# POSTECH-CVLab/PyTorch-StudioGAN

Hardware: AMD Instinct MI355X
Metric: images/sec (G+D step) BigGAN ImageNet-128 bs256 (higher is better)
Workload: dtype bf16

## Files before the change

include/sgamd.h:

```cpp
#ifndef SGAMD_H
#define SGAMD_H
#include <stdint.h>
#ifdef __cplusplus
extern "C" {
#endif

typedef void* sg_stream_t;

#define SG_DTYPE_F32 0
#define SG_DTYPE_BF16 1
#define SG_DTYPE_F64 2

#define SG_PIX_RELU 1
#define SG_PIX_UPSAMPLE 2
#define SG_PIX_QUAD 4
#define SG_PIX_TRANSPOSED 8
#define SG_EPI_OUT_F32 1
#define SG_EPI_ATOMIC 2
#define SG_EPI_POOL 4
#define SG_EPI_RELU 8
#define SG_EPI_RES_F32 16

const char* sg_last_error(void);
int sg_version(void);
// ... 167 lines not shown
  float* sigma;
  float* u_snap; float* v_snap;
  void* w_fwd;
  void* w_dgrad;
  float* w_f32;
  int rows, cols;
  int Cin, RS;
  int do_power_iter;
  int apply_sn;
  int rows_pad;
  long long work_off;
  int trans;
  int dgrad_noflip;
  int Cin_pad;
} sg_sn_layer;
int sg_sn_forward(int dtype, const sg_sn_layer* layers_dev, const sg_sn_layer* layers_host, int n, float eps, float* work, long long work_floats, sg_stream_t s);

typedef struct {
  const float* dwt;
  const float* w;
  const float* u; const float* v; const float* sigma;
  float* dw;
  int rows, cols, Cin, RS, natural, apply_sn, trans;
  int Cin_pad;
} sg_sn_bwd_layer;
int sg_sn_backward(const sg_sn_bwd_layer* layers_dev, const sg_sn_bwd_layer* layers_host, int n, float* work, long long work_floats, sg_stream_t s);

int sg_embedding_fwd(const float* table, const int64_t* idx, float* out, int B, int dim, int num, sg_stream_t s);
int sg_embedding_bwd(const float* dout, const int64_t* idx, float* dtable, int B, int dim, int num, sg_stream_t s);
int sg_relu_sum_hw_fwd(int dtype, const void* x, float* h, int B, int HW, int C, sg_stream_t s);
int sg_relu_sum_hw_bwd(int dtype, const void* x, const float* dh, void* dx, int B, int HW, int C, sg_stream_t s);
int sg_pd_head_fwd(const float* h, const float* w1, const float* b1, const float* emb, float* adv, int B, int C, sg_stream_t s);
int sg_pd_head_bwd(const float* h, const float* w1, const float* emb, const float* dadv, float* dh, float* dw1, float* db1,
                   float* demb, int B, int C, sg_stream_t s);
int sg_loss_d(int kind, const float* real, const float* fake, int B, float* loss, float* d_real, float* d_fake, sg_stream_t s);
int sg_loss_g(int kind, const float* fake, int B, float* loss, float* d_fake, sg_stream_t s);

int sg_interp_rows(const float* real, const float* fake, const float* alpha, float* out, int B, long long n, sg_stream_t s);
int sg_gp_fwd(int kind, const float* grads, int B, long long n, float* norms, float* loss, sg_stream_t s);
int sg_gp_bwd(int kind, const float* grads, const float* norms, const float* gout, float* dgrads, int B, long long n, sg_stream_t s);
int sg_masked_sum_hw(int dtype, const void* t, const void* x, float* out, int B, int HW, int C, sg_stream_t s);

int sg_attn_fwd_flash_ok(int B, int HW, int HW4, int Dp, int Cg);
int sg_attn_fwd_fused(const void* theta, const void* phi, const void* g, float* lse, void* O, float* O32, int B, int HW, int HW4, int Dp, int Cg, sg_stream_t s);
int sg_attn_bwd_fused_ok(int B, int HW, int HW4, int Dp, int Cg);
int sg_attn_bwd_fused(const void* theta, const void* phi, const void* g, const void* dO, const float* O32, const float* lse, float* delta, void* dtheta, void* dphi,
                      void* dg, int B, int HW, int HW4, int Dp, int Cg, sg_stream_t s);

int sg_attn_proj_ok(int B, int H, int W, int C, int ldx, int Dp, int Cg);
int sg_attn_proj_fwd(const void* x, int ldx, const void* w_theta, const void* w_phi, const void* w_g, void* theta, void* phi, void* g,
                     uint8_t* idx_phi, uint8_t* idx_g, int B, int H, int W, int C, int Dp, int Cg, int relu, sg_stream_t s);
int sg_attn_proj_bwd_data(const void* dtheta, const void* dphi, const void* dg, const uint8_t* idx_phi, const uint8_t* idx_g, const void* wd_theta,
                          const void* wd_phi, const void* wd_g, const void* res, void* dx, int B, int H, int W, int C, int Dp, int Cg, sg_stream_t s);

int sg_slice_up_fwd(int dtype, const void* x, void* y, int N, int Hs, int Ws, int ldx, int C, int up, sg_stream_t s);
int sg_slice_up_bwd(int dtype, const void* dy, void* dx, int N, int Hs, int Ws, int ldx, int C, int up, sg_stream_t s);
int sg_copy_channels(int dtype, const void* src, int ld_src, void* dst, int ld_dst, long long rows, int C, sg_stream_t s);

int sg_adam_ema(float* p, const float* g, float* m, float* v, float* ema, long long n, float lr, float beta1, float beta2,
                float eps, float wd, int step, float ema_decay, float grad_scale, sg_stream_t s);
int sg_ema_lerp(const float* src, float* ema, long long n, float decay, sg_stream_t s);

int sg_lecam(const float* real, const float* fake, int B, float ema_real, float ema_fake, float* loss, float* d_real, float* d_fake, sg_stream_t s);
int sg_u8_to_nhwc(int dtype, const uint8_t* x, const uint8_t* flip, void* y, int N, int H, int W, int cpad, sg_stream_t s);

int sg_quantize_resize_normalize(int dtype, const float* x, void* out, uint8_t* quant_out, int N, int C, int H, int W,
                                 int OH, int OW, int quantize, sg_stream_t s);
int sg_quantize_resize_normalize_ms(int dtype, const float* x, void* out, uint8_t* quant_out, int N, int C, int H, int W,
                                    int OH, int OW, int quantize, const float* mean, const float* std, sg_stream_t s);
int sg_pool2d(int dtype, const void* x, void* y, int N, int H, int W, int C, int k, int stride, int pad, int mode, int ldy, int c_off, sg_stream_t s);
int sg_pil_resize_normalize(int dtype, const float* x, void* out, float* tmp, int N, int C, int H, int W, int OH, int OW,
                            const int* bounds_h, const double* kk_h, int ksize_h, const int* bounds_v, const double* kk_v, int ksize_v,
                            int quantize, sg_stream_t s);
int sg_pil_resize_normalize_ms(int dtype, const float* x, void* out, float* tmp, int N, int C, int H, int W, int OH, int OW,
                               const int* bounds_h, const double* kk_h, int ksize_h, const int* bounds_v, const double* kk_v, int ksize_v,
                               int quantize, const float* mean, const float* std, sg_stream_t s);
int sg_global_avgpool(int dtype, const void* x, float* y, int N, int HW, int C, sg_stream_t s);
int sg_topk_hits(const float* scores, int ld, int ncls, const int64_t* labels, int k, int N, uint8_t* hits, sg_stream_t s);
int sg_topk_select(const float* x, int n, int k, float* vals, int* idx, sg_stream_t s);
int sg_topk_scatter(const float* g, const int* idx, int k, float* dx, int n, sg_stream_t s);
int sg_feat_moments_accumulate(const float* f, int n, int C, double* sum_f, double* sum_ff, sg_stream_t s);
int sg_gather_images_u8(const uint8_t* src, const int64_t* idx, const uint8_t* flip, uint8_t* dst, int B, int H, int W,
                        const int64_t* lab_src, int64_t* lab_dst, sg_stream_t s);
int sg_row_normalize_fwd(const float* x, float* y, float* inv, int rows, int cols, float eps, sg_stream_t s);
int sg_row_normalize_bwd(const float* y, const float* inv, const float* dy, float* dx, int rows, int cols, sg_stream_t s);
int sg_row_dot(const float* a, const float* b, float* p, int rows, int cols, sg_stream_t s);
int sg_row_scale(const float* g, const float* x, float* out, int rows, int cols, int accumulate, sg_stream_t s);
int sg_class_loss(int kind, const float* z, const int64_t* label, int rows, int cols, float* row_loss, float* loss, float* dz, sg_stream_t s);
int sg_contrastive_loss(int kind, const float* S, const float* p, const int64_t* label, int B, float temperature, float m_p,
                        float* row_loss, float* loss, float* dS, float* dp, sg_stream_t s);
int sg_gather_cols(const float* z, const int64_t* label, int rows, int cols, float* out, sg_stream_t s);
int sg_scatter_cols(const float* g, const int64_t* label, int rows, int cols, float* dz, sg_stream_t s);
int sg_layernorm_rows(int out_dtype, const float* x, long long pitch, const float* gamma, const float* beta, void* y, long long ldo, int rows, int C,
                      float eps, sg_stream_t s);
int sg_vit_tokens(const float* patch, const float* cls, const float* pos, float* x, int B, int N, int C, sg_stream_t s);
int sg_gelu_f32(const float* x, float* y, long long n, sg_stream_t s);
int sg_tok_gemm(int epi, const void* a, int lda, const void* w, const float* bias, void* out, int ldo, int M, int N, int K, sg_stream_t s);
int sg_mha_fwd_ok(int B, int N, int H, int D);
int sg_mha_fwd(const void* qkv, void* out, int B, int N, int H, int D, float scale, sg_stream_t s);
long long sg_tok_gemm_launches(void);
long long sg_mha_launches(void);

int sg_row_sqnorm(const float* f, int n, int C, float* sq, sg_stream_t s);
int sg_kth_smallest_rows(const float* D, long long ld, int rows, int cols, int k, const float* row_add, float* out, sg_stream_t s);
int sg_prdc_rows(const float* D, long long ld, int rows, int cols, const float* row_add, const float* r2_row, const float* r2_col,
                 int* col_cnt, uint8_t* row_any, float* row_min, sg_stream_t s);
// ... 62 lines not shown
```

pytorch-studiogan_amd/_lib.py:

```python
import ctypes as C
import os
import subprocess
import sys

import torch

_HERE = os.path.dirname(os.path.abspath(__file__))
LIB_PATH = os.path.join(_HERE, "libsgamd.so")
if os.environ.get("SG_LIBSGAMD"):
    LIB_PATH = os.path.abspath(os.environ["SG_LIBSGAMD"])
CSRC = os.path.join(_HERE, "csrc")

F32, BF16, F64 = 0, 1, 2
PIX_RELU, PIX_UPSAMPLE, PIX_QUAD, PIX_TRANSPOSED = 1, 2, 4, 8
Q_POOL, Q_UP = 0, 1
EPI_OUT_F32, EPI_ATOMIC, EPI_POOL, EPI_RELU, EPI_RES_F32 = 1, 2, 4, 8, 16

_vp, _i, _f, _ll = C.c_void_p, C.c_int, C.c_float, C.c_longlong


class ConvFwdDesc(C.Structure):
    _fields_ = [("dtype", _i), ("N", _i), ("Hs", _i), ("Ws", _i), ("C", _i), ("ldx", _i), ("Ho", _i), ("Wo", _i), ("Cout", _i),
                ("R", _i), ("S", _i), ("stride", _i), ("pad_h", _i), ("pad_w", _i), ("pix_flags", _i), ("epi_flags", _i),
                ("alpha", _f), ("beta", _f), ("x", _vp), ("w", _vp), ("bias", _vp), ("res", _vp), ("mask", _vp), ("out", _vp),
# ... 96 lines not shown
    "sg_gemm": [C.POINTER(GemmDesc), _vp],
    "sg_nchw_to_nhwc": [_i, _vp, _vp, _i, _i, _i, _i, _i, _vp],
    "sg_nhwc_to_nchw": [_i, _vp, _vp, _i, _i, _i, _i, _i, _i, _vp],
    "sg_nchw_grad_to_nhwc": [_i, _vp, _vp, _vp, _i, _i, _i, _i, _i, _i, _vp],
    "sg_avgpool2_fwd": [_i, _vp, _vp, _i, _i, _i, _i, _vp],
    "sg_avgpool2_bwd": [_i, _vp, _vp, _i, _i, _i, _i, _vp],
    "sg_maxpool2_fwd": [_i, _vp, _i, _vp, _i, _vp, _i, _i, _i, _i, _vp],
    "sg_maxpool2_bwd": [_i, _vp, _i, _vp, _vp, _i, _i, _i, _i, _i, _vp],
    "sg_softmax_rows": [_i, _vp, _vp, _ll, _i, _vp],
    "sg_softmax_rows_bwd": [_i, _vp, _vp, _vp, _ll, _i, _vp],
    "sg_axpby": [_i, _vp, _vp, _ll, _f, _f, _vp],
    "sg_convert": [_i, _i, _vp, _vp, _ll, _vp],
    "sg_add_relu": [_i, _vp, _vp, _vp, _ll, _vp],
    "sg_relu_mask": [_i, _vp, _vp, _vp, _ll, _vp],
    "sg_dot": [_i, _vp, _vp, _ll, _vp, _f, _vp, _vp],
    "sg_colsum": [_i, _vp, _i, _vp, _i, _ll, _i, _vp, _f, _vp],
    "sg_bn_partial_stats": [_i, _vp, _i, _ll, _i, _vp, _vp],
    "sg_bn_finalize": [_vp, C.c_double, _i, _f, _f, _vp, _vp, _vp, _vp, _vp],
    "sg_comm_unique_id": [_vp],
    "sg_comm_init_rank": [_vp, _i, _i, C.POINTER(_vp)],
    "sg_comm_size": [_vp, C.POINTER(_i)],
    "sg_comm_destroy": [_vp],
    "sg_allreduce_flat": [_vp, _vp, _ll, _i, _vp],
    "sg_bn_stats_sync": [_i, _vp, _i, _ll, _i, _vp, _vp, _f, _f, _vp, _vp, _vp, _vp, _vp],
    "sg_set_f32_mode": [_i],
    "sg_get_f32_mode": [],
    "sg_f32_split_launches": [_i],
    "sg_reduce_scatter_flat": [_vp, _vp, _ll, _vp],
    "sg_allgather_flat": [_vp, _vp, _ll, _vp],
    "sg_p2p_create": [_i, _i, _ll, C.POINTER(_vp), _vp],
    "sg_p2p_connect": [_vp, _vp],
    "sg_p2p_destroy": [_vp],
    "sg_p2p_timeouts": [_vp, C.POINTER(_i)],
    "sg_p2p_allreduce_f64": [_vp, _vp, _i, _vp],
    "sg_bn_finalize_p2p": [_vp, _vp, C.c_double, _i, _f, _f, _vp, _vp, _vp, _vp, _vp],
    "sg_bn_stats_sync_p2p": [_i, _vp, _i, _ll, _i, _vp, _vp, _f, _f, _vp, _vp, _vp, _vp, _vp],
    "sg_bn_from_running": [_vp, _vp, _i, _f, _vp, _vp, _vp],
    "sg_bn_apply": [_i, _vp, _vp, _i, _ll, _i, _vp, _vp, _vp, _vp, _i, _i, _vp],
    "sg_bn_bwd_reduce": [_i, _vp, _vp, _i, _ll, _i, _vp, _vp, _vp, _vp, _i, _i, _vp, _vp],
    "sg_bn_bwd_finalize": [_vp, _i, _i, _vp, _i, _vp, _vp, _vp, _vp],
    "sg_bn_bwd_apply": [_i, _vp, _vp, _vp, _i, _ll, _i, _vp, _vp, _vp, _vp, _i, _i, _vp, C.c_double, _i, _vp],
    "sg_bn_bwd_apply_res": [_i, _vp, _vp, _vp, _i, _ll, _i, _vp, _vp, _vp, _vp, _i, _i, _vp, C.c_double, _i, _vp, _vp],
    "sg_bn_bwd2_reduce": [_i, _vp, _vp, _vp, _i, _ll, _i, _vp, _vp, _vp, _vp, _i, _vp, _vp],
    "sg_bn_bwd2_finalize": [_vp, _i, _i, _vp, _vp],
    "sg_bn_bwd2_dgain": [_vp, _vp, C.c_double, _vp, _i, _i, _vp, _vp],
    "sg_bn_bwd2_apply": [_i, _vp, _vp, _vp, _vp, _vp, _i, _ll, _i, _vp, _vp, _vp, _vp, _i, _vp, C.c_double, _i, _vp],
    "sg_attn_fwd_flash_ok": [_i, _i, _i, _i, _i],
    "sg_attn_fwd_fused": [_vp, _vp, _vp, _vp, _vp, _vp, _i, _i, _i, _i, _i, _vp],
    "sg_attn_bwd_fused_ok": [_i, _i, _i, _i, _i],
    "sg_attn_bwd_fused": [_vp, _vp, _vp, _vp, _vp, _vp, _vp, _vp, _vp, _vp, _i, _i, _i, _i, _i, _vp],
    "sg_attn_proj_ok": [_i, _i, _i, _i, _i, _i, _i],
    "sg_attn_proj_fwd": [_vp, _i, _vp, _vp, _vp, _vp, _vp, _vp, _vp, _vp, _i, _i, _i, _i, _i, _i, _i, _vp],
    "sg_attn_proj_bwd_data": [_vp, _vp, _vp, _vp, _vp, _vp, _vp, _vp, _vp, _vp, _i, _i, _i, _i, _i, _i, _vp],
    "sg_slice_up_fwd": [_i, _vp, _vp, _i, _i, _i, _i, _i, _i, _vp],
    "sg_slice_up_bwd": [_i, _vp, _vp, _i, _i, _i, _i, _i, _i, _vp],
    "sg_copy_channels": [_i, _vp, _i, _vp, _i, _ll, _i, _vp],
    "sg_interp_rows": [_vp, _vp, _vp, _vp, _i, _ll, _vp],
    "sg_gp_fwd": [_i, _vp, _i, _ll, _vp, _vp, _vp],
    "sg_gp_bwd": [_i, _vp, _vp, _vp, _vp, _i, _ll, _vp],
    "sg_masked_sum_hw": [_i, _vp, _vp, _vp, _i, _i, _i, _vp],
    "sg_sn_forward": [_i, _vp, C.POINTER(SnLayer), _i, _f, _vp, _ll, _vp],
    "sg_sn_backward": [_vp, C.POINTER(SnBwdLayer), _i, _vp, _ll, _vp],
    "sg_embedding_fwd": [_vp, _vp, _vp, _i, _i, _i, _vp],
    "sg_embedding_bwd": [_vp, _vp, _vp, _i, _i, _i, _vp],
    "sg_relu_sum_hw_fwd": [_i, _vp, _vp, _i, _i, _i, _vp],
    "sg_relu_sum_hw_bwd": [_i, _vp, _vp, _vp, _i, _i, _i, _vp],
    "sg_pd_head_fwd": [_vp, _vp, _vp, _vp, _vp, _i, _i, _vp],
    "sg_pd_head_bwd": [_vp, _vp, _vp, _vp, _vp, _vp, _vp, _vp, _i, _i, _vp],
    "sg_loss_d": [_i, _vp, _vp, _i, _vp, _vp, _vp, _vp],
    "sg_loss_g": [_i, _vp, _i, _vp, _vp, _vp],
    "sg_adam_ema": [_vp, _vp, _vp, _vp, _vp, _ll, _f, _f, _f, _f, _f, _i, _f, _f, _vp],
    "sg_ema_lerp": [_vp, _vp, _ll, _f, _vp],
    "sg_quantize_resize_normalize": [_i, _vp, _vp, _vp, _i, _i, _i, _i, _i, _i, _i, _vp],
    "sg_pil_resize_normalize": [_i, _vp, _vp, _vp, _i, _i, _i, _i, _i, _i, _vp, _vp, _i, _vp, _vp, _i, _i, _vp],
    "sg_quantize_resize_normalize_ms": [_i, _vp, _vp, _vp, _i, _i, _i, _i, _i, _i, _i, C.POINTER(_f), C.POINTER(_f), _vp],
    "sg_pil_resize_normalize_ms": [_i, _vp, _vp, _vp, _i, _i, _i, _i, _i, _i, _vp, _vp, _i, _vp, _vp, _i, _i, C.POINTER(_f), C.POINTER(_f), _vp],
    "sg_layernorm_rows": [_i, _vp, _ll, _vp, _vp, _vp, _ll, _i, _i, _f, _vp],
    "sg_vit_tokens": [_vp, _vp, _vp, _vp, _i, _i, _i, _vp],
    "sg_gelu_f32": [_vp, _vp, _ll, _vp],
    "sg_tok_gemm": [_i, _vp, _i, _vp, _vp, _vp, _i, _i, _i, _i, _vp],
    "sg_mha_fwd_ok": [_i, _i, _i, _i],
    "sg_mha_fwd": [_vp, _vp, _i, _i, _i, _i, _f, _vp],
    "sg_tok_gemm_launches": [],
    "sg_mha_launches": [],
    "sg_pool2d": [_i, _vp, _vp, _i, _i, _i, _i, _i, _i, _i, _i, _i, _i, _vp],
    "sg_global_avgpool": [_i, _vp, _vp, _i, _i, _i, _vp],
    "sg_feat_moments_accumulate": [_vp, _i, _i, _vp, _vp, _vp],
    "sg_topk_hits": [_vp, _i, _i, _vp, _i, _i, _vp, _vp],
    "sg_row_normalize_fwd": [_vp, _vp, _vp, _i, _i, _f, _vp],
    "sg_row_normalize_bwd": [_vp, _vp, _vp, _vp, _i, _i, _vp],
    "sg_row_dot": [_vp, _vp, _vp, _i, _i, _vp],
    "sg_row_scale": [_vp, _vp, _vp, _i, _i, _i, _vp],
    "sg_class_loss": [_i, _vp, _vp, _i, _i, _vp, _vp, _vp, _vp],
    "sg_contrastive_loss": [_i, _vp, _vp, _vp, _i, _f, _f, _vp, _vp, _vp, _vp, _vp],
    "sg_gather_cols": [_vp, _vp, _i, _i, _vp, _vp],
    "sg_scatter_cols": [_vp, _vp, _i, _i, _vp, _vp],
    "sg_chol_lower": [_vp, _i, _vp, _vp],
    "sg_dgemm_tn": [_vp, _vp, _vp, _i, _vp],
    "sg_jacobi_sweep": [_vp, _i, _vp, _vp],
    "sg_row_norm_sum": [_vp, _i, _vp, _vp],
    "sg_row_sqnorm": [_vp, _i, _i, _vp, _vp],
    "sg_kth_smallest_rows": [_vp, _ll, _i, _i, _i, _vp, _vp, _vp],
    "sg_prdc_rows": [_vp, _ll, _i, _i, _vp, _vp, _vp, _vp, _vp, _vp, _vp],
    "sg_topk_select": [_vp, _i, _i, _vp, _vp, _vp],
    "sg_lecam": [_vp, _vp, _i, _f, _f, _vp, _vp, _vp, _vp],
    "sg_u8_to_nhwc": [_i, _vp, _vp, _vp, _i, _i, _i, _i, _vp],
# ... 114 lines not shown
```

pytorch-studiogan_amd/csrc/attn_proj.hip:

```cpp
#include <stdlib.h>
#include "common.h"
#include "../../include/sgamd.h"

namespace {

constexpr unsigned OOR = 0x80000000u;

typedef short s16x2_t __attribute__((ext_vector_type(2)));

__device__ __forceinline__ unsigned quad_pixel(int row, int H, int W, int wshift, int hshift) {
  const int qd = row >> 2, dy = (row >> 1) & 1, dx = row & 1;
  const int wq = qd & ((W >> 1) - 1);
  const int t = qd >> (wshift - 1);
  const int hq = t & ((H >> 1) - 1);
  const int n = t >> (hshift - 1);
  return (unsigned)(n * H + 2 * hq + dy) * (unsigned)W + (unsigned)(2 * wq + dx);
}

struct ApFwdParams {
  const bf16_t* x; const bf16_t* wt; const bf16_t* wp; const bf16_t* wg;
  bf16_t* theta; bf16_t* phi; bf16_t* g; uint8_t* iphi; uint8_t* ig;
  int C, ldx, H, W, wshift, hshift, J, relu, nrb;
  unsigned xbytes, tbytes, pbytes, gbytes;
};
// ... 261 lines not shown
#pragma unroll
        for (int it = 0; it < NIT; it++) {
          const int idx = lane + 64 * it;
          const int r = idx / CPR, c = idx - r * CPR;
          if (idx < 32 * CPR) *(u32x4*)(stg + r * CP + c * 16) = pre[it];
        }
        asm volatile("s_waitcnt lgkmcnt(0)" ::: "memory");
      }
#pragma unroll
      for (int a = 0; a < TI; a++)
#pragma unroll
        for (int g4 = 0; g4 < 4; g4++) {
          const int il = a * 32 + 8 * g4 + 4 * fhi;
          char* loc = stg + frow * CP + il * 2;
          float v[4] = {acc[a][4 * g4 + 0], acc[a][4 * g4 + 1], acc[a][4 * g4 + 2], acc[a][4 * g4 + 3]};
          if (pre_res) {
            const u32x2 r = *(const u32x2*)loc;
#pragma unroll
            for (int e = 0; e < 4; e++) v[e] += bf2f((bf16_t)((r[e >> 1] >> (16 * (e & 1))) & 0xffffu));
          }
          u32x2 t;
          t[0] = pack2bf(v[0], v[1]);
          t[1] = pack2bf(v[2], v[3]);
          *(u32x2*)loc = t;
        }
      asm volatile("s_waitcnt lgkmcnt(0)" ::: "memory");
#pragma unroll
      for (int it = 0; it < NIT; it++) {
        const int idx = lane + 64 * it;
        const int r = idx / CPR, c = idx - r * CPR;
        const int row = rb * 32 + r;
        const bool ok = idx < 32 * CPR && row < p.J && c < ncp;
        const unsigned off = ok ? quad_pixel(row, p.H, p.W, p.wshift, p.hshift) * C2 + (unsigned)(ic0 + c * 8) * 2u : OOR;
        const u32x4 v = *(const u32x4*)(stg + (r & 31) * CP + c * 16);
        __builtin_amdgcn_raw_buffer_store_b128(v, rso, (int)off, 0, 0);
      }
    }
  };

  const int stride = gridDim.x * NW;
  int rb = blockIdx.x * NW + wave;
  if (rb >= p.nrb) return;
  Frag fa, fb;
  fetch(rb, fa);
  while (true) {
    fetch(rb + stride, fb);
    compute_store(rb, fa);
    rb += stride;
    if (rb >= p.nrb) break;
    fetch(rb + stride, fa);
    compute_store(rb, fb);
    rb += stride;
    if (rb >= p.nrb) break;
  }
}

int ilog2_pow2(int v) {
  if (v <= 0 || (v & (v - 1))) return -1;
  int s = 0;
  while ((1 << s) < v) s++;
  return s;
}
bool al16(const void* p) { return (((uintptr_t)p) & 15) == 0; }

int family(int C, int Dp, int Cg) {
  if (Dp == 16 && Cg == 48 && C <= 96) return 0;
  if (Dp == 24 && Cg == 96 && C <= 192) return 1;
  return -1;
}

template <typename K> int set_lds(K kern, int lds) {
  return hipFuncSetAttribute((const void*)kern, hipFuncAttributeMaxDynamicSharedMemorySize, lds) == hipSuccess ? 0 : -1;
}

}

extern "C" int sg_attn_proj_ok(int B, int H, int W, int C, int ldx, int Dp, int Cg) {
  if (B <= 0 || ilog2_pow2(H) < 1 || ilog2_pow2(W) < 1 || C <= 0 || C % 8 || ldx % 8 || ldx < C) return 0;
  if (family(C, Dp, Cg) < 0) return 0;
  const long long J = (long long)B * H * W;
  if (J >= (1ll << 30) || J * ldx * 2 >= (1ll << 31) || J * C * 2 >= (1ll << 31)) return 0;
  return 1;
}

extern "C" int sg_attn_proj_fwd(const void* x, int ldx, const void* w_theta, const void* w_phi, const void* w_g, void* theta, void* phi, void* g,
                                uint8_t* idx_phi, uint8_t* idx_g, int B, int H, int W, int C, int Dp, int Cg, int relu, sg_stream_t s) {
  SG_CHECK(x && w_theta && w_phi && w_g && theta && phi && g && idx_phi && idx_g, "sg_attn_proj_fwd: null");
  SG_CHECK(sg_attn_proj_ok(B, H, W, C, ldx, Dp, Cg) == 1, "sg_attn_proj_fwd: unsupported shape (ask sg_attn_proj_ok)");
  SG_CHECK(al16(x) && al16(w_theta) && al16(w_phi) && al16(w_g) && al16(theta) && al16(phi) && al16(g) && !(((uintptr_t)idx_phi | (uintptr_t)idx_g) & 7),
           "sg_attn_proj_fwd: misaligned pointer");
  hipStream_t st = (hipStream_t)s;
  ApFwdParams p;
  p.x = (const bf16_t*)x; p.wt = (const bf16_t*)w_theta; p.wp = (const bf16_t*)w_phi; p.wg = (const bf16_t*)w_g;
  p.theta = (bf16_t*)theta; p.phi = (bf16_t*)phi; p.g = (bf16_t*)g; p.iphi = idx_phi; p.ig = idx_g;
  p.C = C; p.ldx = ldx; p.H = H; p.W = W; p.wshift = ilog2_pow2(W); p.hshift = ilog2_pow2(H);
  const long long J = (long long)B * H * W;
  p.J = (int)J; p.relu = relu ? 1 : 0; p.nrb = (int)((J + 31) / 32);
  p.xbytes = (unsigned)(((J - 1) * ldx + C) * 2); p.tbytes = (unsigned)(J * Dp * 2); p.pbytes = (unsigned)(J / 4 * Dp * 2); p.gbytes = (unsigned)(J / 4 * Cg * 2);
  const double I = 2.0 * Dp + Cg;
  const int prof = sg_prof_begin(st, 2.0 * I * (double)J * (double)C, 0);
  sg_prof_tag(prof, SG_ENG_CONV_SK, 2.0 * ((double)J * C + I * C + (double)J * Dp) + 0.25 * (double)J * (Dp + Cg) * 3.0);
#define AP_FWD(DP8, CG8, KS, NW)                                                                                     \
  {                                                                                                                  \
    constexpr int NT = ((2 * DP8 + CG8) * 8 + 31) / 32;                                                              \
    constexpr int lds = NT * 32 * (KS * 32 + 16) + NW * 32 * (NT * 64 + 16);                                         \
    static_assert(lds <= 160 * 1024, "LDS");                                                                         \
    static bool done = false;                                                                                        \
    if (!done) { SG_CHECK(set_lds(k_attn_proj_fwd<DP8, CG8, KS, NW>, lds) == 0, "sg_attn_proj_fwd: LDS attribute"); done = true; } \
    int gx = (p.nrb + NW - 1) / NW;                                                                                  \
    const int cap = 256 * (8 / NW);                                                                                  \
    if (gx > cap) gx = cap;                                                                                          \
    hipLaunchKernelGGL((k_attn_proj_fwd<DP8, CG8, KS, NW>), dim3(gx), dim3(64 * NW), lds, st, p);                    \
  }
  if (family(C, Dp, Cg) == 0) AP_FWD(2, 6, 6, 4) else AP_FWD(3, 12, 12, 8)
#undef AP_FWD
  sg_prof_end(st, prof);
  SG_LAUNCH_CHECK();
  return 0;
}

extern "C" int sg_attn_proj_bwd_data(const void* dtheta, const void* dphi, const void* dg, const uint8_t* idx_phi, const uint8_t* idx_g, const void* wd_theta,
                                     const void* wd_phi, const void* wd_g, const void* res, void* dx, int B, int H, int W, int C, int Dp, int Cg, sg_stream_t s) {
  SG_CHECK(dtheta && dphi && dg && idx_phi && idx_g && wd_theta && wd_phi && wd_g && dx, "sg_attn_proj_bwd_data: null");
  SG_CHECK(sg_attn_proj_ok(B, H, W, C, C, Dp, Cg) == 1, "sg_attn_proj_bwd_data: unsupported shape (ask sg_attn_proj_ok)");
  SG_CHECK(al16(dtheta) && al16(dphi) && al16(dg) && al16(wd_theta) && al16(wd_phi) && al16(wd_g) && al16(res) && al16(dx) &&
           !(((uintptr_t)idx_phi | (uintptr_t)idx_g) & 7), "sg_attn_proj_bwd_data: misaligned pointer");
  hipStream_t st = (hipStream_t)s;
  ApBwdParams p;
  p.dtheta = (const bf16_t*)dtheta; p.dphi = (const bf16_t*)dphi; p.dg = (const bf16_t*)dg; p.iphi = idx_phi; p.ig = idx_g;
  p.wt = (const bf16_t*)wd_theta; p.wp = (const bf16_t*)wd_phi; p.wg = (const bf16_t*)wd_g;
  p.res = (const bf16_t*)res; p.dx = (bf16_t*)dx;
  p.C = C; p.H = H; p.W = W; p.wshift = ilog2_pow2(W); p.hshift = ilog2_pow2(H);
  const long long J = (long long)B * H * W;
  p.J = (int)J; p.nrb = (int)((J + 31) / 32);
  p.tbytes = (unsigned)(J * Dp * 2); p.pbytes = (unsigned)(J / 4 * Dp * 2); p.gbytes = (unsigned)(J / 4 * Cg * 2); p.obytes = (unsigned)(J * C * 2);
  const double I = 2.0 * Dp + Cg;
  const int prof = sg_prof_begin(st, 2.0 * I * (double)J * (double)C, 0);
  sg_prof_tag(prof, SG_ENG_CONV_SK, 2.0 * ((double)J * C * (res ? 2.0 : 1.0) + I * C + (double)J * Dp) + 0.25 * (double)J * (Dp + Cg) * 3.0);
#define AP_BWD(DP8, CG8, TI, NP, NW)                                                                                 \
  {                                                                                                                  \
    constexpr int KS = 2 * ((DP8 + 1) / 2) + CG8 / 2;                                                                \
    constexpr int lds = TI * NP * 32 * (KS * 32 + 16) + NW * 32 * (TI * 64 + 16);                                    \
    static_assert(lds <= 160 * 1024, "LDS");                                                                         \
    static bool done = false;                                                                                        \
    if (!done) { SG_CHECK(set_lds(k_attn_proj_bwd<DP8, CG8, TI, NP, NW>, lds) == 0, "sg_attn_proj_bwd_data: LDS attribute"); done = true; } \
    int gx = (p.nrb + NW - 1) / NW;                                                                                  \
    const int cap = 256 * (8 / NW);                                                                                  \
    if (gx > cap) gx = cap;                                                                                          \
    hipLaunchKernelGGL((k_attn_proj_bwd<DP8, CG8, TI, NP, NW>), dim3(gx), dim3(64 * NW), lds, st, p);                \
  }
  if (family(C, Dp, Cg) == 0) AP_BWD(2, 6, 3, 1, 4) else AP_BWD(3, 12, 3, 2, 8)
#undef AP_BWD
  sg_prof_end(st, prof);
  SG_LAUNCH_CHECK();
  return 0;
}
```

pytorch-studiogan_amd/functional/attention.py:

```python
from ._base import *
from .layout import ConvertFn
from .conv import ConvCfg, ConvDgradFn, ConvFn, _conv_wgrad

class MaxPool2Fn(torch.autograd.Function):

    @staticmethod
    def forward(ctx, x):
        x = _c(x)
        B, H, W, Cc = x.shape
        y = torch.empty((B, (H // 2) * (W // 2), Cc), dtype=x.dtype, device=x.device)
        idx = torch.empty((B, (H // 2) * (W // 2), Cc), dtype=torch.uint8, device=x.device)
        L.call("sg_maxpool2_fwd", L.dt(x), L.ptr(x), Cc, L.ptr(y), Cc, L.ptr(idx), B, H, W, Cc, L.stream())
        ctx.save_for_backward(idx)
        ctx.dims = (B, H, W, Cc)
        return y

    @staticmethod
    def backward(ctx, dy):
        (idx,) = ctx.saved_tensors
        if torch.is_grad_enabled():
            return MaxPool2BwdFn.apply(dy, idx, ctx.dims)
        return _maxpool2_bwd(dy, idx, ctx.dims)


# ... 156 lines not shown
        P = lse = o32 = None
        o = torch.empty((B, H, W, Cg), dtype=T, device=dev)
        if fused:
            lse = torch.empty((B, HW), dtype=torch.float32, device=dev)
            o32 = torch.empty((B, HW, Cg), dtype=torch.float32, device=dev) if need_grad else None
            L.call("sg_attn_fwd_fused", L.ptr(theta), L.ptr(phi), L.ptr(g), L.ptr(lse), L.ptr(o), L.ptr(o32), B, HW, HW4, Dp, Cg, L.stream())
        else:
            S = torch.empty((B, HW, HW4), dtype=torch.float32, device=dev)
            gemm_raw(sd, phi, 0, Dp, theta, 0, Dp, S, HW4, HW4, HW, Dp, batch=B, p_bs=HW4 * Dp, q_bs=HW * Dp, out_bs=HW * HW4, epi_flags=L.EPI_OUT_F32)
            P = torch.empty((B, HW, HW4), dtype=T, device=dev)
            L.call("sg_softmax_rows", sd, L.ptr(S), L.ptr(P), B * HW, HW4, L.stream())
            del S
            gemm_raw(sd, g, 1, Cg, P, 0, HW4, o, Cg, Cg, HW, HW4, batch=B, p_bs=HW4 * Cg, q_bs=HW * HW4, out_bs=HW * Cg)
        ctx.save_for_backward(theta, phi, g, P, lse, o32)
        ctx.dims = (B, H, W, Dp, Cg)
        return o

    @staticmethod
    def backward(ctx, do):
        theta, phi, g, P, lse, o32 = ctx.saved_tensors
        B, H, W, Dp, Cg = ctx.dims
        if torch.is_grad_enabled():
            with torch.enable_grad():
                ins = [t for t, need in zip((theta, phi, g), ctx.needs_input_grad) if need]
                grads = list(torch.autograd.grad(_attn_reference_graph(theta, phi, g, ctx.dims), ins, do, create_graph=True)) if ins else []
            return tuple(grads.pop(0) if need else None for need in ctx.needs_input_grad)
        HW, HW4 = H * W, (H // 2) * (W // 2)
        do = _c(do)
        dev, T = do.device, do.dtype
        sd = L.dt(T)
        dtheta = torch.empty((B, H, W, Dp), dtype=T, device=dev)
        dphi = torch.empty((B, HW4, Dp), dtype=T, device=dev)
        dg = torch.empty((B, HW4, Cg), dtype=T, device=dev)
        if P is None:
            delta = torch.empty((B, HW), dtype=torch.float32, device=dev)
            L.call("sg_attn_bwd_fused", L.ptr(theta), L.ptr(phi), L.ptr(g), L.ptr(do), L.ptr(o32), L.ptr(lse), L.ptr(delta), L.ptr(dtheta), L.ptr(dphi),
                   L.ptr(dg), B, HW, HW4, Dp, Cg, L.stream())
            return dtheta, dphi, dg
        gemm_raw(sd, do, 1, Cg, P, 1, HW4, dg, Cg, Cg, HW4, HW, batch=B, p_bs=HW * Cg, q_bs=HW * HW4, out_bs=HW4 * Cg)
        dP = torch.empty((B, HW, HW4), dtype=torch.float32, device=dev)
        gemm_raw(sd, g, 0, Cg, do, 0, Cg, dP, HW4, HW4, HW, Cg, batch=B, p_bs=HW4 * Cg, q_bs=HW * Cg, out_bs=HW * HW4, epi_flags=L.EPI_OUT_F32)
        dS = torch.empty((B, HW, HW4), dtype=T, device=dev)
        L.call("sg_softmax_rows_bwd", sd, L.ptr(P), L.ptr(dP), L.ptr(dS), B * HW, HW4, L.stream())
        del dP
        gemm_raw(sd, phi, 1, Dp, dS, 0, HW4, dtheta, Dp, Dp, HW, HW4, batch=B, p_bs=HW4 * Dp, q_bs=HW * HW4, out_bs=HW * Dp)
        gemm_raw(sd, theta, 1, Dp, dS, 1, HW4, dphi, Dp, Dp, HW4, HW, batch=B, p_bs=HW * Dp, q_bs=HW * HW4, out_bs=HW4 * Dp)
        return dtheta, dphi, dg


def attn_proj_on():
    return os.environ.get("SG_ATTN_PROJ", "1") != "0"


def attn_proj_ok(x, rts):
    rt_t, rt_p, rt_g = rts
    if x.dtype != torch.bfloat16 or x.dim() != 4 or rt_t.rows_pad != rt_p.rows_pad or any(r.RS != 1 or r.trans or r.cin_pad != x.shape[3] for r in rts):
        return False
    B, H, W, Cc = x.shape
    return L.lib().sg_attn_proj_ok(B, H, W, Cc, Cc, rt_t.rows_pad, rt_g.rows_pad) == 1


class AttnProjFn(torch.autograd.Function):

    @staticmethod
    def forward(ctx, x, w_theta, w_phi, w_g, rts, slot, link=None):
        x = _c(x)
        rt_t, rt_p, rt_g = rts
        bank = rt_t.bank()
        B, H, W, Cc = x.shape
        Dp, Cg = rt_t.rows_pad, rt_g.rows_pad
        ctx.link = link
        if link is not None and link.chain:
            link.pending += 1
        for _ in rts:
            _tick()
        HW4 = (H // 2) * (W // 2)
        theta = torch.empty((B, H, W, Dp), dtype=x.dtype, device=x.device)
        phi = torch.empty((B, HW4, Dp), dtype=x.dtype, device=x.device)
        g = torch.empty((B, HW4, Cg), dtype=x.dtype, device=x.device)
        iphi = torch.empty((B, HW4, Dp), dtype=torch.uint8, device=x.device)
        ig = torch.empty((B, HW4, Cg), dtype=torch.uint8, device=x.device)
        L.call("sg_attn_proj_fwd", L.ptr(x), Cc, bank.w_fwd(slot, rt_t), bank.w_fwd(slot, rt_p), bank.w_fwd(slot, rt_g), L.ptr(theta), L.ptr(phi), L.ptr(g),
               L.ptr(iphi), L.ptr(ig), B, H, W, Cc, Dp, Cg, 0, L.stream())
        ctx.save_for_backward(x, iphi, ig)
        ctx.rts, ctx.slot = rts, slot
        ctx.weights = (w_theta, w_phi, w_g)
        return theta, phi, g

    @staticmethod
    def backward(ctx, dtheta, dphi, dg):
        x, iphi, ig = ctx.saved_tensors
        rts, slot = ctx.rts, ctx.slot
        B, H, W, Cc = x.shape
        cfg = ConvCfg(1, 1)
        if torch.is_grad_enabled():
            if not ctx.needs_input_grad[0]:
                return (None,) * 7
            with torch.enable_grad():
                outs = (ConvFn.apply(x, ctx.weights[0], None, None, rts[0], slot, cfg, None),
                        MaxPool2Fn.apply(ConvFn.apply(x, ctx.weights[1], None, None, rts[1], slot, cfg, None)),
                        MaxPool2Fn.apply(ConvFn.apply(x, ctx.weights[2], None, None, rts[2], slot, cfg, None)))
                (dx,) = torch.autograd.grad(outs, [x], [dtheta, dphi, dg], create_graph=True)
            return (dx,) + (None,) * 6
        bank = rts[0].bank()
        Dp, Cg = rts[0].rows_pad, rts[2].rows_pad
        dtheta, dphi, dg = _c(dtheta), _c(dphi), _c(dg)
        dx = None
        skip_dx = ctx.link.take() if ctx.link is not None else None
        if ctx.needs_input_grad[0]:
            dx = torch.empty_like(x)
            L.call("sg_attn_proj_bwd_data", L.ptr(dtheta), L.ptr(dphi), L.ptr(dg), L.ptr(iphi), L.ptr(ig), bank.w_dgrad(slot, rts[0]), bank.w_dgrad(slot, rts[1]),
                   bank.w_dgrad(slot, rts[2]), L.ptr(skip_dx), L.ptr(dx), B, H, W, Cc, Dp, Cg, L.stream())
        elif skip_dx is not None:
            raise RuntimeError("GradLink: a residual gradient was handed over but the attention block's input needs no gradient")
        if ctx.link is not None and ctx.link.chain:
            ctx.link.pending -= 1
        for k, (dy, idx) in enumerate(((dtheta, None), (dphi, iphi), (dg, ig))):
            if ctx.needs_input_grad[1 + k]:
                full = dy if idx is None else _maxpool2_bwd(dy, idx, (B, H, W, dy.shape[-1]))
                _conv_wgrad(x, full, rts[k], slot, cfg)
        return (dx,) + (None,) * 6


class AttnOutFn(torch.autograd.Function):

    @staticmethod
    def forward(ctx, x, o, weight, sigma, rt, slot, link=None):
        bank = rt.bank()
        x, o = _c(x), _c(o)
        ctx.link = link
        y = conv2d_raw(o, bank.w_fwd(slot, rt), rt.Cin, rt.rows, 1, 1, res=x, alpha_ptr=sigma)
        ctx.save_for_backward(o, sigma)
        ctx.rt, ctx.slot = rt, slot
        ctx.sigma_param = sigma
        ctx.weight = weight
        return y

    @staticmethod
    def backward(ctx, dy):
        o, sigma = ctx.saved_tensors
        rt, slot = ctx.rt, ctx.slot
        if torch.is_grad_enabled():
            if _param_grad_wanted(ctx.weight, ctx.sigma_param):
                raise NotImplementedError("create_graph=True is supported for input gradients only (WGAN-GP / R1 path)")
            do = ScalePtrFn.apply(ConvDgradFn.apply(dy, o, ctx.weight, rt, slot, ConvCfg(1, 1)), ctx.sigma_param) if ctx.needs_input_grad[1] else None
            return (dy if ctx.needs_input_grad[0] else None), do, None, None, None, None, None
        bank = rt.bank()
        dy = _c(dy)
        N, H, W, Cc = dy.shape
        do = None
        if ctx.needs_input_grad[3]:
            t = conv2d_raw(o, bank.w_fwd(slot, rt), rt.Cin, rt.rows, 1, 1)
            g = ensure_grad(ctx.sigma_param)
            L.call("sg_dot", L.dt(dy), L.ptr(dy), L.ptr(t), dy.numel(), L.ptr(g), 1.0, None, L.stream())
        if ctx.needs_input_grad[1]:
            do = conv2d_raw(dy, bank.w_dgrad(slot, rt), rt.rows, rt.Cin, 1, 1, alpha_ptr=sigma)
        if ctx.needs_input_grad[2]:
            conv2d_wgrad_raw(o, dy, bank.dwt(slot, rt), rt.Cin, rt.rows, 1, 1, H, W, alpha_ptr=sigma)
        dx = dy
        if ctx.link is not None and ctx.link.pending > 0 and ctx.needs_input_grad[0]:
            ctx.link.dx, dx = dy, None
        return dx, do, None, None, None, None, None


__all__ = ['AttnCoreFn', 'AttnOutFn', 'AttnPooledFn', 'AttnProjFn', 'attn_proj_ok', 'attn_proj_on', 'BmmFn', 'MaxPool2BwdFn', 'MaxPool2Fn', 'ScalePtrFn', 'SoftmaxRowsBwdFn', 'SoftmaxRowsFn', '_attn_reference_graph', '_maxpool2_bwd']
```

Before: 2081.

## Fuse attention projection weight gradients with inline max-unpool into one kernel

Adds a fused HIP kernel that computes the weight gradients of the theta, phi and g 1x1 projections in a single pass over the input. It unpools the pooled phi/g gradients in LDS using the stored argmax indices, instead of materialising full-resolution gradients and running three separate wgrad convolutions. Each workgroup writes its partial sums to a float workspace, and a second kernel reduces them into the weight-gradient buffers. This is meant to cut repeated reads of x, the unpool kernels and extra launches, at the cost of a per-call workspace allocation and a split-K reduction pass.

```diff
diff --git a/include/sgamd.h b/include/sgamd.h
--- a/include/sgamd.h
+++ b/include/sgamd.h
@@ -243,6 +243,10 @@
                      uint8_t* idx_phi, uint8_t* idx_g, int B, int H, int W, int C, int Dp, int Cg, int relu, sg_stream_t s);
 int sg_attn_proj_bwd_data(const void* dtheta, const void* dphi, const void* dg, const uint8_t* idx_phi, const uint8_t* idx_g, const void* wd_theta,
                           const void* wd_phi, const void* wd_g, const void* res, void* dx, int B, int H, int W, int C, int Dp, int Cg, sg_stream_t s);
+int sg_attn_proj_wgrad_plan(int B, int H, int W, int C, int Dp, int Cg, long long* work_floats);
+int sg_attn_proj_wgrad(const void* x, int ldx, const void* dtheta, const void* dphi, const void* dg, const uint8_t* idx_phi, const uint8_t* idx_g,
+                       float* dw_theta, float* dw_phi, float* dw_g, float* work, long long work_floats, int B, int H, int W, int C, int Dp, int Cg,
+                       sg_stream_t s);
 
 int sg_slice_up_fwd(int dtype, const void* x, void* y, int N, int Hs, int Ws, int ldx, int C, int up, sg_stream_t s);
 int sg_slice_up_bwd(int dtype, const void* dy, void* dx, int N, int Hs, int Ws, int ldx, int C, int up, sg_stream_t s);
diff --git a/pytorch-studiogan_amd/_lib.py b/pytorch-studiogan_amd/_lib.py
--- a/pytorch-studiogan_amd/_lib.py
+++ b/pytorch-studiogan_amd/_lib.py
@@ -172,6 +172,8 @@
     "sg_attn_proj_ok": [_i, _i, _i, _i, _i, _i, _i],
     "sg_attn_proj_fwd": [_vp, _i, _vp, _vp, _vp, _vp, _vp, _vp, _vp, _vp, _i, _i, _i, _i, _i, _i, _i, _vp],
     "sg_attn_proj_bwd_data": [_vp, _vp, _vp, _vp, _vp, _vp, _vp, _vp, _vp, _vp, _i, _i, _i, _i, _i, _i, _vp],
+    "sg_attn_proj_wgrad_plan": [_i, _i, _i, _i, _i, _i, C.POINTER(_ll)],
+    "sg_attn_proj_wgrad": [_vp, _i, _vp, _vp, _vp, _vp, _vp, _vp, _vp, _vp, _vp, _ll, _i, _i, _i, _i, _i, _i, _vp],
     "sg_slice_up_fwd": [_i, _vp, _vp, _i, _i, _i, _i, _i, _i, _vp],
     "sg_slice_up_bwd": [_i, _vp, _vp, _i, _i, _i, _i, _i, _i, _vp],
     "sg_copy_channels": [_i, _vp, _i, _vp, _i, _ll, _i, _vp],
diff --git a/pytorch-studiogan_amd/csrc/attn_proj.hip b/pytorch-studiogan_amd/csrc/attn_proj.hip
--- a/pytorch-studiogan_amd/csrc/attn_proj.hip
+++ b/pytorch-studiogan_amd/csrc/attn_proj.hip
@@ -337,6 +337,220 @@
     compute_store(rb, fb);
     rb += stride;
     if (rb >= p.nrb) break;
+  }
+}
+
+struct ApWgParams {
+  const bf16_t* x; const bf16_t* dtheta; const bf16_t* dphi; const bf16_t* dg; const uint8_t* iphi; const uint8_t* ig;
+  float* work;
+  int C, ldx, H, W, wshift, hshift, J, nchunk;
+  unsigned xbytes, tbytes;
+};
+
+__device__ __forceinline__ bf16x8_t ap_tr_frag(const char* img, int pitch, int row0, int ks, int lane) {
+  typedef __attribute__((address_space(3))) s16x4 lds_s16x4;
+  const int g16 = lane >> 4, t = lane & 15;
+  const char* p = img + (ks * 16 + 8 * (g16 >> 1) + (t >> 2)) * pitch + (row0 + 16 * (g16 & 1) + 4 * (t & 3)) * 2;
+  const s16x4 a = __builtin_amdgcn_ds_read_tr16_b64_v4i16((lds_s16x4*)p);
+  const s16x4 b = __builtin_amdgcn_ds_read_tr16_b64_v4i16((lds_s16x4*)(p + 4 * pitch));
+  s16x8 r;
+  r[0] = a[0]; r[1] = a[1]; r[2] = a[2]; r[3] = a[3];
+  r[4] = b[0]; r[5] = b[1]; r[6] = b[2]; r[7] = b[3];
+  return __builtin_bit_cast(bf16x8_t, r);
+}
+
+template <int DP8, int CG8, int NH>
+__global__ __launch_bounds__(256) void k_attn_proj_wgrad(ApWgParams p) {
+  constexpr int I = (2 * DP8 + CG8) * 8;
+  constexpr int NJ = (I + 31) / 32;
+  constexpr int NI = 3;
+  constexpr int XC = NI * 4;
+  constexpr int XP = NI * 64, GP = NJ * 64;
+  constexpr int WSZ = 32 * (XP + GP);
+  constexpr int PCH = DP8 + CG8;
+  constexpr int NX = 32 * XC / 64, NT = (32 * DP8 + 63) / 64, NP = (8 * PCH + 63) / 64;
+  constexpr int NG = 4 / NH;
+  extern __shared__ __attribute__((aligned(16))) char smem[];
+  const int tid = threadIdx.x, lane = tid & 63;
+  const int wave = __builtin_amdgcn_readfirstlane(tid >> 6);
+  const int half = wave % NH, grp = wave / NH;
+  char* const xs = smem + wave * WSZ;
+  char* const gs = xs + 32 * XP;
+
+  const auto rsx = __builtin_amdgcn_make_buffer_rsrc((void*)p.x, 0, (int)p.xbytes, 0x00020000);
+  const auto rst = __builtin_amdgcn_make_buffer_rsrc((void*)p.dtheta, 0, (int)p.tbytes, 0x00020000);
+  const unsigned ldx2 = 2u * (unsigned)p.ldx;
+  const int JQ = p.J >> 2;
+
+  for (int o = lane * 16; o < 32 * GP; o += 1024) *(u32x4*)(gs + o) = (u32x4){0u, 0u, 0u, 0u};
+
+  struct Regs { u32x4 x[NX]; u32x4 t[NT]; u32x4 pg[NP]; u32x2 pi[NP]; };
+
+  auto fetch = [&](int c, Regs& f) {
+    const bool cok = c < p.nchunk;
+#pragma unroll
+    for (int j = 0; j < NX; j++) {
+      const int idx = lane + 64 * j;
+      const int px = idx / XC, cb = idx - px * XC;
+      const int row = c * 32 + px, ch = half * (NI * 32) + cb * 8;
+      const unsigned off = (cok && row < p.J && ch < p.C) ? quad_pixel(row, p.H, p.W, p.wshift, p.hshift) * ldx2 + (unsigned)ch * 2u : OOR;
+      f.x[j] = __builtin_bit_cast(u32x4, __builtin_amdgcn_raw_buffer_load_b128(rsx, (int)off, 0, 0));
+    }
+#pragma unroll
+    for (int j = 0; j < NT; j++) {
+      const int idx = lane + 64 * j;
+      const int px = idx / DP8, cb = idx - px * DP8;
+      const int row = c * 32 + px;
+      const unsigned off = (cok && idx < 32 * DP8 && row < p.J) ? (quad_pixel(row, p.H, p.W, p.wshift, p.hshift) * DP8 + (unsigned)cb) * 16u : OOR;
+      f.t[j] = __builtin_bit_cast(u32x4, __builtin_amdgcn_raw_buffer_load_b128(rst, (int)off, 0, 0));
+    }
+#pragma unroll
+    for (int j = 0; j < NP; j++) {
+      const int idx = lane + 64 * j;
+      const int qw = idx / PCH, cv = idx - qw * PCH;
+      const int Q = c * 8 + qw;
+      const bool ok = cok && idx < 8 * PCH && Q < JQ;
+      const bool isphi = cv < DP8;
+      const bf16_t* gp = !ok ? p.dphi : isphi ? p.dphi + ((long long)Q * DP8 + cv) * 8 : p.dg + ((long long)Q * CG8 + (cv - DP8)) * 8;
+      f.pg[j] = *(const u32x4*)gp;
+      const uint8_t* ip = !ok ? p.iphi : isphi ? p.iphi + ((long long)Q * DP8 + cv) * 8 : p.ig + ((long long)Q * CG8 + (cv - DP8)) * 8;
+      f.pi[j] = *(const u32x2*)ip;
+    }
+  };
+
+  auto unpool = [](u32x4 g, u32x2 av, uint32_t pos) {
+    u32x4 o;
+#pragma unroll
+    for (int d = 0; d < 4; d++) {
+      const uint32_t w = d < 2 ? av[0] : av[1];
+      const uint32_t a0 = (w >> (16 * (d & 1))) & 0xffu, a1 = (w >> (16 * (d & 1) + 8)) & 0xffu;
+      o[d] = (a0 == pos ? (g[d] & 0xffffu) : 0u) | (a1 == pos ? (g[d] & 0xffff0000u) : 0u);
+    }
+    return o;
+  };
+
+  f32x16 acc[NI][NJ];
+#pragma unroll
+  for (int a = 0; a < NI; a++)
+#pragma unroll
+    for (int b = 0; b < NJ; b++)
+#pragma unroll
+      for (int r = 0; r < 16; r++) acc[a][b][r] = 0.f;
+
+  auto stage = [&](int c, const Regs& f) {
+    asm volatile("s_waitcnt lgkmcnt(0)" ::: "memory");
+#pragma unroll
+    for (int j = 0; j < NX; j++) {
+      const int idx = lane + 64 * j;
+      const int px = idx / XC, cb = idx - px * XC;
+      *(u32x4*)(xs + px * XP + cb * 16) = f.x[j];
+    }
+#pragma unroll
+    for (int j = 0; j < NT; j++) {
+      const int idx = lane + 64 * j;
+      const int px = idx / DP8, cb = idx - px * DP8;
+      if (idx < 32 * DP8) *(u32x4*)(gs + px * GP + cb * 16) = f.t[j];
+    }
+#pragma unroll
+    for (int j = 0; j < NP; j++) {
+      const int idx = lane + 64 * j;
+      const int qw = idx / PCH, cv = idx - qw * PCH;
+      if (idx < 8 * PCH) {
+        const u32x4 v = (c < p.nchunk && c * 8 + qw < JQ) ? f.pg[j] : (u32x4){0u, 0u, 0u, 0u};
+#pragma unroll
+        for (int pos = 0; pos < 4; pos++) *(u32x4*)(gs + (4 * qw + pos) * GP + (DP8 + cv) * 16) = unpool(v, f.pi[j], (uint32_t)pos);
+      }
+    }
+    asm volatile("s_waitcnt lgkmcnt(0)" ::: "memory");
+  };
+
+  auto multiply = [&]() {
+#pragma unroll
+    for (int ks = 0; ks < 2; ks++) {
+      bf16x8_t af[NI], bf[NJ];
+#pragma unroll
+      for (int a = 0; a < NI; a++) af[a] = ap_tr_frag(xs, XP, a * 32, ks, lane);
+#pragma unroll
+      for (int b = 0; b < NJ; b++) bf[b] = ap_tr_frag(gs, GP, b * 32, ks, lane);
+#pragma unroll
+      for (int a = 0; a < NI; a++)
+#pragma unroll
+        for (int b = 0; b < NJ; b++) acc[a][b] = __builtin_amdgcn_mfma_f32_32x32x16_bf16(af[a], bf[b], acc[a][b], 0, 0, 0);
+    }
+  };
+
+  const int nstream = gridDim.x * NG;
+  int c = blockIdx.x * NG + grp;
+  if (c < p.nchunk) {
+    Regs fa, fb;
+    fetch(c, fa);
+    fetch(c + nstream, fb);
+    for (; c < p.nchunk; c += 2 * nstream) {
+      stage(c, fa);
+      fetch(c + 2 * nstream, fa);
+      multiply();
+      stage(c + nstream, fb);
+      fetch(c + 3 * nstream, fb);
+      multiply();
+    }
+  }
+
+  float* const red = (float*)smem + half * (NI * NJ * 4 * 256);
+  float* const out = p.work + (long long)blockIdx.x * ((long long)I * p.C);
+#pragma unroll 1
+  for (int r = 0; r < NG; r++) {
+    __syncthreads();
+    if (grp != r) continue;
+#pragma unroll
+    for (int a = 0; a < NI; a++)
+#pragma unroll
+      for (int b = 0; b < NJ; b++) {
+        asm volatile("" ::: "memory");
+#pragma unroll
+        for (int g4 = 0; g4 < 4; g4++) {
+          f32x4 v = {acc[a][b][4 * g4 + 0], acc[a][b][4 * g4 + 1], acc[a][b][4 * g4 + 2], acc[a][b][4 * g4 + 3]};
+          f32x4* const loc = (f32x4*)(red + (((a * NJ + b) * 4 + g4) * 64 + lane) * 4);
+          if (r > 0) v += *loc;
+          if (r < NG - 1) { *loc = v; continue; }
+          const int jrow = b * 32 + (lane & 31);
+          const int ch = half * (NI * 32) + a * 32 + 8 * g4 + 4 * (lane >> 5);
+          if (jrow < I && ch < p.C) *(f32x4*)(out + (long long)jrow * p.C + ch) = v;
+        }
+      }
+  }
+}
+
+__global__ __launch_bounds__(256) void k_attn_proj_wgrad_reduce(const float* partial, int splits, long long n, float* o0, float* o1, float* o2, long long n0, long long n1) {
+  __shared__ f32x4 sm[4][64];
+  const long long nt4 = n >> 2;
+  const int li = threadIdx.x & 63, q = threadIdx.x >> 6;
+  for (long long i0 = blockIdx.x * 64ll; i0 < nt4; i0 += (long long)gridDim.x * 64) {
+    const long long i = i0 + li;
+    f32x4 a[8];
+#pragma unroll
+    for (int k = 0; k < 8; k++) a[k] = (f32x4){0.f, 0.f, 0.f, 0.f};
+    if (i < nt4) {
+      const float* src = partial + 4 * i;
+      int s = q;
+      for (; s + 28 < splits; s += 32) {
+        f32x4 v[8];
+#pragma unroll
+        for (int k = 0; k < 8; k++) v[k] = *(const f32x4*)(src + (long long)(s + 4 * k) * n);
+#pragma unroll
+        for (int k = 0; k < 8; k++) a[k] += v[k];
+      }
+      for (; s < splits; s += 4) a[0] += *(const f32x4*)(src + (long long)s * n);
+    }
+    sm[q][li] = ((a[0] + a[1]) + (a[2] + a[3])) + ((a[4] + a[5]) + (a[6] + a[7]));
+    __syncthreads();
+    if (q == 0 && i < nt4) {
+      const f32x4 t = (sm[0][li] + sm[1][li]) + (sm[2][li] + sm[3][li]);
+      const long long e = 4 * i;
+      float* dst = e < n0 ? o0 + e : e < n0 + n1 ? o1 + (e - n0) : o2 + (e - n0 - n1);
+      const f32x4 o = *(f32x4*)dst;
+      *(f32x4*)dst = o + t;
+    }
+    __syncthreads();
   }
 }
 
@@ -440,3 +654,58 @@
   SG_LAUNCH_CHECK();
   return 0;
 }
+
+static int ap_wgrad_nwg(long long J, int fam) {
+  const long long nchunk = (J + 31) / 32, ng = fam == 0 ? 4 : 2;
+  const long long nwg = (nchunk + ng - 1) / ng;
+  return (int)(nwg > 256 ? 256 : nwg);
+}
+
+extern "C" int sg_attn_proj_wgrad_plan(int B, int H, int W, int C, int Dp, int Cg, long long* work_floats) {
+  SG_CHECK(work_floats, "sg_attn_proj_wgrad_plan: null");
+  SG_CHECK(sg_attn_proj_ok(B, H, W, C, C, Dp, Cg) == 1, "sg_attn_proj_wgrad_plan: unsupported shape (ask sg_attn_proj_ok)");
+  *work_floats = (long long)ap_wgrad_nwg((long long)B * H * W, family(C, Dp, Cg)) * (2 * Dp + Cg) * C;
+  return 0;
+}
+
+extern "C" int sg_attn_proj_wgrad(const void* x, int ldx, const void* dtheta, const void* dphi, const void* dg, const uint8_t* idx_phi, const uint8_t* idx_g,
+                                  float* dw_theta, float* dw_phi, float* dw_g, float* work, long long work_floats, int B, int H, int W, int C, int Dp, int Cg,
+                                  sg_stream_t s) {
+  SG_CHECK(x && dtheta && dphi && dg && idx_phi && idx_g && dw_theta && dw_phi && dw_g && work, "sg_attn_proj_wgrad: null");
+  SG_CHECK(sg_attn_proj_ok(B, H, W, C, ldx, Dp, Cg) == 1, "sg_attn_proj_wgrad: unsupported shape (ask sg_attn_proj_ok)");
+  SG_CHECK(al16(x) && al16(dtheta) && al16(dphi) && al16(dg) && al16(dw_theta) && al16(dw_phi) && al16(dw_g) && al16(work) &&
+           !(((uintptr_t)idx_phi | (uintptr_t)idx_g) & 7), "sg_attn_proj_wgrad: misaligned pointer");
+  const int fam = family(C, Dp, Cg);
+  const long long J = (long long)B * H * W;
+  const int nwg = ap_wgrad_nwg(J, fam);
+  const long long n = (long long)(2 * Dp + Cg) * C;
+  SG_CHECK(work_floats >= nwg * n, "sg_attn_proj_wgrad: workspace smaller than sg_attn_proj_wgrad_plan asks for");
+  hipStream_t st = (hipStream_t)s;
+  ApWgParams p;
+  p.x = (const bf16_t*)x; p.dtheta = (const bf16_t*)dtheta; p.dphi = (const bf16_t*)dphi; p.dg = (const bf16_t*)dg; p.iphi = idx_phi; p.ig = idx_g;
+  p.work = work;
+  p.C = C; p.ldx = ldx; p.H = H; p.W = W; p.wshift = ilog2_pow2(W); p.hshift = ilog2_pow2(H);
+  p.J = (int)J; p.nchunk = (int)((J + 31) / 32);
+  p.xbytes = (unsigned)(((J - 1) * ldx + C) * 2); p.tbytes = (unsigned)(J * Dp * 2);
+  const double I = 2.0 * Dp + Cg;
+  const int prof = sg_prof_begin(st, 2.0 * I * (double)J * (double)C, 1);
+  sg_prof_tag(prof, SG_ENG_WGRAD_SK, 2.0 * ((double)J * C + (double)J * Dp) + 0.25 * (double)J * (Dp + Cg) * 3.0 + 8.0 * I * C);
+#define AP_WG(DP8, CG8, NH)                                                                                          \
+  {                                                                                                                  \
+    constexpr int NJ = ((2 * DP8 + CG8) * 8 + 31) / 32;                                                              \
+    constexpr int stage = 4 * 32 * (3 * 64 + NJ * 64), red = NH * 3 * NJ * 4096;                                     \
+    constexpr int lds = stage > red ? stage : red;                                                                   \
+    static_assert(lds <= 160 * 1024, "LDS");                                                                         \
+    static bool done = false;                                                                                        \
+    if (!done) { SG_CHECK(set_lds(k_attn_proj_wgrad<DP8, CG8, NH>, lds) == 0, "sg_attn_proj_wgrad: LDS attribute"); done = true; } \
+    hipLaunchKernelGGL((k_attn_proj_wgrad<DP8, CG8, NH>), dim3(nwg), dim3(256), lds, st, p);                         \
+  }
+  if (fam == 0) AP_WG(2, 6, 1) else AP_WG(3, 12, 2)
+#undef AP_WG
+  long long blocks = (n / 4 + 63) / 64;
+  hipLaunchKernelGGL(k_attn_proj_wgrad_reduce, dim3((int)blocks), dim3(256), 0, st, (const float*)work, nwg, n, dw_theta, dw_phi, dw_g, (long long)Dp * C,
+                     (long long)Dp * C);
+  sg_prof_end(st, prof);
+  SG_LAUNCH_CHECK();
+  return 0;
+}
diff --git a/pytorch-studiogan_amd/functional/attention.py b/pytorch-studiogan_amd/functional/attention.py
--- a/pytorch-studiogan_amd/functional/attention.py
+++ b/pytorch-studiogan_amd/functional/attention.py
@@ -232,6 +232,10 @@
     return os.environ.get("SG_ATTN_PROJ", "1") != "0"
 
 
+def attn_proj_wgrad_on():
+    return attn_proj_on() and os.environ.get("SG_ATTN_PROJ_WGRAD", "1") != "0"
+
+
 def attn_proj_ok(x, rts):
     rt_t, rt_p, rt_g = rts
     if x.dtype != torch.bfloat16 or x.dim() != 4 or rt_t.rows_pad != rt_p.rows_pad or any(r.RS != 1 or r.trans or r.cin_pad != x.shape[3] for r in rts):
@@ -295,6 +299,14 @@
             raise RuntimeError("GradLink: a residual gradient was handed over but the attention block's input needs no gradient")
         if ctx.link is not None and ctx.link.chain:
             ctx.link.pending -= 1
+        if all(ctx.needs_input_grad[1:4]) and attn_proj_wgrad_on():
+            assert cfg.scale == 1.0
+            wf = L.C.c_longlong(0)
+            L.call("sg_attn_proj_wgrad_plan", B, H, W, Cc, Dp, Cg, L.C.byref(wf))
+            work = torch.empty(wf.value, dtype=torch.float32, device=x.device)
+            L.call("sg_attn_proj_wgrad", L.ptr(x), Cc, L.ptr(dtheta), L.ptr(dphi), L.ptr(dg), L.ptr(iphi), L.ptr(ig), bank.dwt(slot, rts[0]), bank.dwt(slot, rts[1]),
+                   bank.dwt(slot, rts[2]), L.ptr(work), wf.value, B, H, W, Cc, Dp, Cg, L.stream())
+            return (dx,) + (None,) * 6
         for k, (dy, idx) in enumerate(((dtheta, None), (dphi, iphi), (dg, ig))):
             if ctx.needs_input_grad[1 + k]:
                 full = dy if idx is None else _maxpool2_bwd(dy, idx, (B, H, W, dy.shape[-1]))
@@ -343,4 +355,4 @@
         return dx, do, None, None, None, None, None
 
 
-__all__ = ['AttnCoreFn', 'AttnOutFn', 'AttnPooledFn', 'AttnProjFn', 'attn_proj_ok', 'attn_proj_on', 'BmmFn', 'MaxPool2BwdFn', 'MaxPool2Fn', 'ScalePtrFn', 'SoftmaxRowsBwdFn', 'SoftmaxRowsFn', '_attn_reference_graph', '_maxpool2_bwd']
+__all__ = ['AttnCoreFn', 'AttnOutFn', 'AttnPooledFn', 'AttnProjFn', 'attn_proj_ok', 'attn_proj_on', 'attn_proj_wgrad_on', 'BmmFn', 'MaxPool2BwdFn', 'MaxPool2Fn', 'ScalePtrFn', 'SoftmaxRowsBwdFn', 'SoftmaxRowsFn', '_attn_reference_graph', '_maxpool2_bwd']
```

After: 2098 (median of 6 runs). Within noise of the previous version (+0.8%).
